# vinits5/bullet-envs

Measured on AMD Instinct MI355X. Metric: env-steps/sec (whole node), 16-link snake, 4096 envs/GPU, higher is better.
Workload: dtype f32

## Files before the change

### bullet-envs_amd/csrc/snk_dynamics.hpp

```cpp
#pragma once
#include "snk_lds.hpp"
#include "snk_model.hpp"
#include "snk_wave.hpp"

namespace snk {

#ifndef SNK_SCALAR_DYNAMICS
__device__ __forceinline__ float quad_yzx(float x) {
    return __int_as_float(__builtin_amdgcn_update_dpp(0, __float_as_int(x), 0xC9, 0xf, 0xf, true));
}
__device__ __forceinline__ float quad_zxy(float x) {
    return __int_as_float(__builtin_amdgcn_update_dpp(0, __float_as_int(x), 0xD2, 0xf, 0xf, true));
}
__device__ __forceinline__ float lane_cross(float a_yzx, float a_zxy, float b) {
#pragma clang fp contract(off)
    return __builtin_fmaf(a_yzx, quad_zxy(b), -(a_zxy * quad_yzx(b)));
}
struct LaneVel {
    float w, v, za, zl;
};
__device__ __forceinline__ LaneVel lane_vel_step(float wp, float vp, float ax, float rb, float qdb) {
#pragma clang fp contract(off)
    const float wy = quad_yzx(wp), wz = quad_zxy(wp);
    const float cr = lane_cross(wy, wz, rb);
    LaneVel o;
    o.w = __builtin_fmaf(ax, qdb, wp);
    o.v = vp + cr;
    o.za = lane_cross(wy, wz, ax) * qdb;
    o.zl = lane_cross(wy, wz, cr);
    return o;
}
#endif

template <class LT>
__device__ void fk_vel(LT& L, const DevModel& M, int lane) {
    constexpr int N = LT::kN;
    const float* bs = L.base();
    float qx = bs[3], qy = bs[4], qz = bs[5], qw = bs[6];
    float dd = qx * qx + qy * qy + qz * qz + qw * qw;
    float s2 = 2.0f / dd;
    float xs = qx * s2, ys = qy * s2, zs = qz * s2;
    float wx = qw * xs, wy = qw * ys, wz = qw * zs;
    float xx = qx * xs, xy = qx * ys, xz = qx * zs, yy = qy * ys, yz = qy * zs, zz = qz * zs;
    float Rp[9] = {1 - (yy + zz), xy - wz, xz + wy, xy + wz, 1 - (xx + zz), yz - wx, xz - wy, yz + wx, 1 - (xx + yy)};
    f3 op = ld3(bs), wp = ld3(bs + 7), vp = ld3(bs + 10);
    if (lane == 0) {
#pragma unroll
        for (int i = 0; i < 9; i++) L.R[0][i] = Rp[i];
        st3(L.o[0], op); st3(L.w[0], wp); st3(L.v[0], vp);
        st3(L.r[0], mk3(0, 0, 0)); st3(L.ax[0], mk3(0, 0, 0));
#pragma unroll
        for (int i = 0; i < 6; i++) L.zeta[0][i] = 0.f;
    }
    float snv = 0.f, csv = 1.f;
    if (lane < N) sincosf(L.q()[lane], &snv, &csv);
#ifndef SNK_SCALAR_DYNAMICS
    const int ln = launder_lane(lane);
    const int c = ln & 3, cc = c < 3 ? c : 2;
    float C0 = c == 0 ? Rp[0] : (c == 1 ? Rp[3] : Rp[6]);
    float C1 = c == 0 ? Rp[1] : (c == 1 ? Rp[4] : Rp[7]);
    float C2 = c == 0 ? Rp[2] : (c == 1 ? Rp[5] : Rp[8]);
    float opv = bs[cc], wpv = bs[7 + cc], vpv = bs[10 + cc];
#pragma unroll 4
    for (int b = 1; b <= N; b++) {
#pragma clang fp contract(off)
        const float* Rf = M.Rfix[b];
        const float* pf = M.pfix[b];
        const float qdb = L.qd()[b - 1];
        const float sn = __int_as_float(__builtin_amdgcn_readlane(__float_as_int(snv), b - 1));
        const float cs = __int_as_float(__builtin_amdgcn_readlane(__float_as_int(csv), b - 1));
        const float T0 = __builtin_fmaf(C2, Rf[6], __builtin_fmaf(C0, Rf[0], C1 * Rf[3]));
        const float T1 = __builtin_fmaf(C2, Rf[7], __builtin_fmaf(C0, Rf[1], C1 * Rf[4]));
        const float T2 = __builtin_fmaf(C2, Rf[8], __builtin_fmaf(C0, Rf[2], C1 * Rf[5]));
        const float N0 = __builtin_fmaf(T0, cs, -(sn * T2));
        const float N2 = __builtin_fmaf(sn, T0, cs * T2);
        const float rb = __builtin_fmaf(C2, pf[2], __builtin_fmaf(C0, pf[0], C1 * pf[1]));
        const float o = opv + rb;
        const LaneVel k = lane_vel_step(wpv, vpv, T1, rb, qdb);
        if (ln < 3) {
            L.R[b][3 * c] = N0; L.R[b][3 * c + 1] = T1; L.R[b][3 * c + 2] = N2;
            L.o[b][c] = o; L.r[b][c] = rb; L.ax[b][c] = T1; L.w[b][c] = k.w; L.v[b][c] = k.v;
            L.zeta[b][c] = k.za; L.zeta[b][3 + c] = k.zl;
        }
        C0 = N0; C1 = T1; C2 = N2;
        opv = o; wpv = k.w; vpv = k.v;
    }
#else
#pragma unroll 4
    for (int b = 1; b <= N; b++) {
        const float* Rf = M.Rfix[b];
        float T[9];
#pragma unroll
        for (int i = 0; i < 3; i++)
#pragma unroll
            for (int j = 0; j < 3; j++)
                T[3 * i + j] = Rp[3 * i] * Rf[j] + Rp[3 * i + 1] * Rf[3 + j] + Rp[3 * i + 2] * Rf[6 + j];
        float qdb = L.qd()[b - 1];
        const float sn = __int_as_float(__builtin_amdgcn_readlane(__float_as_int(snv), b - 1));
        const float cs = __int_as_float(__builtin_amdgcn_readlane(__float_as_int(csv), b - 1));
        float Rn[9];
#pragma unroll
        for (int i = 0; i < 3; i++) {
            Rn[3 * i + 0] = cs * T[3 * i] - sn * T[3 * i + 2];
            Rn[3 * i + 1] = T[3 * i + 1];
            Rn[3 * i + 2] = sn * T[3 * i] + cs * T[3 * i + 2];
        }
        f3 rb = mulRv(Rp, ld3(M.pfix[b]));
        f3 o = op + rb;
        f3 ax = mk3(T[1], T[4], T[7]);
        f3 w = wp + ax * qdb;
        f3 v = vp + cross(wp, rb);
        f3 za = cross(wp, ax) * qdb;
        f3 zl = cross(wp, cross(wp, rb));
        if (lane == 0) {
#pragma unroll
            for (int i = 0; i < 9; i++) L.R[b][i] = Rn[i];
            st3(L.o[b], o); st3(L.r[b], rb); st3(L.ax[b], ax); st3(L.w[b], w); st3(L.v[b], v);
            st3(&L.zeta[b][0], za); st3(&L.zeta[b][3], zl);
        }
#pragma unroll
        for (int i = 0; i < 9; i++) Rp[i] = Rn[i];
        op = o; wp = w; vp = v;
    }
#endif
    lds_sync();
}

template <class LT>
__device__ __forceinline__ void vel_refresh(LT& L, int lane) {
    constexpr int N = LT::kN;
#ifdef SNK_SCALAR_DYNAMICS
    f3 wp = ld3(L.base() + 7), vp = ld3(L.base() + 10);
    if (lane == 0) { st3(L.w[0], wp); st3(L.v[0], vp); }
    for (int b = 1; b <= N; b++) {
        f3 ax = ld3(L.ax[b]), rb = ld3(L.r[b]);
        float qdb = L.qd()[b - 1];
        f3 w = wp + ax * qdb, v = vp + cross(wp, rb);
        f3 za = cross(wp, ax) * qdb, zl = cross(wp, cross(wp, rb));
        if (lane == 0) { st3(L.w[b], w); st3(L.v[b], v); st3(&L.zeta[b][0], za); st3(&L.zeta[b][3], zl); }
        wp = w; vp = v;
    }
#else
    const int ln = launder_lane(lane);
    const int c = ln & 3, cc = c < 3 ? c : 2;
    float wpv = L.base()[7 + cc], vpv = L.base()[10 + cc];
    if (ln < 3) { L.w[0][c] = wpv; L.v[0][c] = vpv; }
    for (int b = 1; b <= N; b++) {
        const LaneVel k = lane_vel_step(wpv, vpv, L.ax[b][cc], L.r[b][cc], L.qd()[b - 1]);
        if (ln < 3) { L.w[b][c] = k.w; L.v[b][c] = k.v; L.zeta[b][c] = k.za; L.zeta[b][3 + c] = k.zl; }
        wpv = k.w; vpv = k.v;
    }
#endif
}

template <class LT>
__device__ float mean_height(LT& L, const DevModel& M, int lane) {
    constexpr int N = LT::kN;
    float z = 0.f;
    if (lane == 0) z = L.o[0][2] + L.R[0][6] * M.hbase[0] + L.R[0][7] * M.hbase[1] + L.R[0][8] * M.hbase[2];
    else if (lane <= N) z = L.o[lane][2];
    return wave_sum<64>(z) * (1.0f / (N + 1));
}

template <class LT, bool FIRST>
__device__ void body_bias(LT& L, const DevModel& M, int lane) {
    constexpr int N = LT::kN;
    if (lane <= N) {
        const int b = lane;
        const float* R = L.R[b];
        f3 w = ld3(L.w[b]), v = ld3(L.v[b]);
        float m = M.mass[b];
        f3 cw = mulRv(R, ld3(M.com[b]));
        float Ibar[6];
        rotSym(R, M.Ib[b], Ibar);
        f3 pN = cross(w, mulSv(Ibar, w));
        f3 pF = cross(w, cross(w, cw)) * m;
        float Irw[6];
        rotSym(R, M.Irot[b], Irw);
        float nw = sqrtf(dot(w, w));
        pN = pN + mulSv(Irw, w) * (M.ang_damp + M.ang_damp * nw);
        const int ns = M.nsub[b];
        for (int s = 0; s < ns; s++) {
            f3 cs = mulRv(R, ld3(M.sub_c[b][s]));
            f3 vs = v + cross(w, cs);
            float nv = sqrtf(dot(vs, vs));
            f3 F = vs * (M.sub_m[b][s] * (M.lin_damp + M.lin_damp * nv));
            pF = pF + F;
            pN = pN + cross(cs, F);
        }
        if (FIRST) {
            f3 G = mk3(0.f, 0.f, m * M.gz);
            pF = pF - G;
            pN = pN - cross(cw, G);
            st3(L.cw[b], cw);
            float* IA = L.IA[b];
#pragma unroll
            for (int i = 0; i < 6; i++) IA[i] = Ibar[i];
            float hx = m * cw.x, hy = m * cw.y, hz = m * cw.z;
            IA[6] = 0.f; IA[7] = -hz; IA[8] = hy;
            IA[9] = hz;  IA[10] = 0.f; IA[11] = -hx;
            IA[12] = -hy; IA[13] = hx; IA[14] = 0.f;
            IA[15] = m; IA[16] = 0.f; IA[17] = 0.f; IA[18] = m; IA[19] = 0.f; IA[20] = m;
        } else {
            pN = pN - ld3(L.ext(b));
            pF = pF - ld3(L.ext(b) + 3);
        }
        st3(&L.p[b][0], pN);
        st3(&L.p[b][3], pF);
    }
}

template <class LT, bool FACTOR>
__device__ void aba_main(LT& L, const DevModel& M, int lane
#ifdef SNK_PROFILE_FINE
                         , unsigned long long* prof_f = nullptr
#endif
) {
    constexpr int N = LT::kN;
    float cA[6], cB[9], cC[6];
#pragma unroll
    for (int i = 0; i < 6; i++) { cA[i] = 0.f; cC[i] = 0.f; }
#pragma unroll
    for (int i = 0; i < 9; i++) cB[i] = 0.f;
    f3 cN = mk3(0, 0, 0), cF = mk3(0, 0, 0);
    for (int b = N; b >= 1; b--) {
        float A[6], B[9], C[6];
        float* IA = L.IA[b];
#pragma unroll
        for (int i = 0; i < 6; i++) { A[i] = IA[i]; C[i] = IA[15 + i]; }
#pragma unroll
        for (int i = 0; i < 9; i++) B[i] = IA[6 + i];
        if (FACTOR) {
#pragma unroll
            for (int i = 0; i < 6; i++) { A[i] += cA[i]; C[i] += cC[i]; }
#pragma unroll
            for (int i = 0; i < 9; i++) B[i] += cB[i];
        }
        f3 pN = ld3(&L.p[b][0]) + cN, pF = ld3(&L.p[b][3]) + cF;
        f3 ax = ld3(L.ax[b]);
        f3 Ua, Ub;
        float Dinv;
        if (FACTOR) {
            Ua = mulSv(A, ax);
            Ub = mk3(B[0] * ax.x + B[3] * ax.y + B[6] * ax.z, B[1] * ax.x + B[4] * ax.y + B[7] * ax.z,
                     B[2] * ax.x + B[5] * ax.y + B[8] * ax.z);
            Dinv = 1.0f / dot(ax, Ua);
        } else {
            Ua = ld3(L.Ua[b]); Ub = ld3(L.Ub[b]); Dinv = L.Dinv[b];
        }
        f3 za = ld3(&L.zeta[b][0]), zl = ld3(&L.zeta[b][3]);
        float u = L.tauj[b - 1] - dot(ax, pN);
        f3 tN = mulSv(A, za) + mk3(B[0] * zl.x + B[1] * zl.y + B[2] * zl.z, B[3] * zl.x + B[4] * zl.y + B[5] * zl.z,
                                   B[6] * zl.x + B[7] * zl.y + B[8] * zl.z);
        f3 tF = mk3(B[0] * za.x + B[3] * za.y + B[6] * za.z, B[1] * za.x + B[4] * za.y + B[7] * za.z,
                    B[2] * za.x + B[5] * za.y + B[8] * za.z) + mulSv(C, zl);
        float uz = dot(Ua, za) + dot(Ub, zl);
        float s = (u - uz) * Dinv;
        f3 paN = pN + tN + Ua * s, paF = pF + tF + Ub * s;
        f3 r = ld3(L.r[b]);
        cN = paN + cross(r, paF);
        cF = paF;
        if (lane == 0) {
            L.u[b] = u;
            if (FACTOR) {
#pragma unroll
                for (int i = 0; i < 6; i++) { IA[i] = A[i]; IA[15 + i] = C[i]; }
#pragma unroll
                for (int i = 0; i < 9; i++) IA[6 + i] = B[i];
                st3(L.Ua[b], Ua); st3(L.Ub[b], Ub); L.Dinv[b] = Dinv;
            }
        }
        if (FACTOR) {
            float ua[3] = {Ua.x, Ua.y, Ua.z}, ub[3] = {Ub.x, Ub.y, Ub.z};
            float Ap[6], Bp[9], Cp[6];
            Ap[0] = A[0] - ua[0] * ua[0] * Dinv; Ap[1] = A[1] - ua[0] * ua[1] * Dinv; Ap[2] = A[2] - ua[0] * ua[2] * Dinv;
            Ap[3] = A[3] - ua[1] * ua[1] * Dinv; Ap[4] = A[4] - ua[1] * ua[2] * Dinv; Ap[5] = A[5] - ua[2] * ua[2] * Dinv;
            Cp[0] = C[0] - ub[0] * ub[0] * Dinv; Cp[1] = C[1] - ub[0] * ub[1] * Dinv; Cp[2] = C[2] - ub[0] * ub[2] * Dinv;
            Cp[3] = C[3] - ub[1] * ub[1] * Dinv; Cp[4] = C[4] - ub[1] * ub[2] * Dinv; Cp[5] = C[5] - ub[2] * ub[2] * Dinv;
#pragma unroll
            for (int i = 0; i < 3; i++)
#pragma unroll
                for (int j = 0; j < 3; j++) Bp[3 * i + j] = B[3 * i + j] - ua[i] * ub[j] * Dinv;
            f3 c0 = cross(r, mk3(Cp[0], Cp[1], Cp[2]));
            f3 c1 = cross(r, mk3(Cp[1], Cp[3], Cp[4]));
            f3 c2 = cross(r, mk3(Cp[2], Cp[4], Cp[5]));
            float Bn[9] = {Bp[0] + c0.x, Bp[1] + c1.x, Bp[2] + c2.x, Bp[3] + c0.y, Bp[4] + c1.y, Bp[5] + c2.y,
                           Bp[6] + c0.z, Bp[7] + c1.z, Bp[8] + c2.z};
            f3 e0 = cross(r, mk3(Bp[0], Bp[1], Bp[2])), e1 = cross(r, mk3(Bp[3], Bp[4], Bp[5])),
               e2 = cross(r, mk3(Bp[6], Bp[7], Bp[8]));
            f3 g0 = cross(r, mk3(Bn[0], Bn[1], Bn[2])), g1 = cross(r, mk3(Bn[3], Bn[4], Bn[5])),
               g2 = cross(r, mk3(Bn[6], Bn[7], Bn[8]));
            cA[0] = Ap[0] + e0.x + g0.x;
            cA[1] = Ap[1] + e0.y + g1.x;
            cA[2] = Ap[2] + e0.z + g2.x;
            cA[3] = Ap[3] + e1.y + g1.y;
            cA[4] = Ap[4] + e1.z + g2.y;
            cA[5] = Ap[5] + e2.z + g2.z;
#pragma unroll
            for (int i = 0; i < 9; i++) cB[i] = Bn[i];
#pragma unroll
            for (int i = 0; i < 6; i++) cC[i] = Cp[i];
        }
    }
    SNK_FSTAMP(2)
    f3 pN = ld3(&L.p[0][0]) + cN, pF = ld3(&L.p[0][3]) + cF;
    float p0[6] = {pN.x, pN.y, pN.z, pF.x, pF.y, pF.z};
    if (FACTOR) {
        float* IA = L.IA[0];
        float A[6], B[9], C[6];
#pragma unroll
        for (int i = 0; i < 6; i++) { A[i] = IA[i] + cA[i]; C[i] = IA[15 + i] + cC[i]; }
#pragma unroll
        for (int i = 0; i < 9; i++) B[i] = IA[6 + i] + cB[i];
        float G[6][6];
        G[0][0] = A[0]; G[0][1] = A[1]; G[0][2] = A[2]; G[1][1] = A[3]; G[1][2] = A[4]; G[2][2] = A[5];
        G[1][0] = A[1]; G[2][0] = A[2]; G[2][1] = A[4];
        G[3][3] = C[0]; G[3][4] = C[1]; G[3][5] = C[2]; G[4][4] = C[3]; G[4][5] = C[4]; G[5][5] = C[5];
        G[4][3] = C[1]; G[5][3] = C[2]; G[5][4] = C[4];
#pragma unroll
        for (int i = 0; i < 3; i++)
#pragma unroll
            for (int j = 0; j < 3; j++) { G[i][3 + j] = B[3 * i + j]; G[3 + j][i] = B[3 * i + j]; }
        float V[6][6];
#pragma unroll
        for (int i = 0; i < 6; i++)
#pragma unroll
            for (int j = 0; j < 6; j++) V[i][j] = (i == j) ? 1.f : 0.f;
#pragma unroll
        for (int k = 0; k < 6; k++) {
            float piv = 1.0f / G[k][k];
#pragma unroll
            for (int j = 0; j < 6; j++) { G[k][j] *= piv; V[k][j] *= piv; }
#pragma unroll
            for (int i = 0; i < 6; i++) {
                if (i != k) {
                    float f = G[i][k];
#pragma unroll
                    for (int j = 0; j < 6; j++) { G[i][j] -= f * G[k][j]; V[i][j] -= f * V[k][j]; }
                }
            }
        }
        if (lane == 0) {
#pragma unroll
            for (int i = 0; i < 6; i++)
#pragma unroll
                for (int j = 0; j < 6; j++) L.Inv0[6 * i + j] = V[i][j];
        }
        float a0[6];
#pragma unroll
        for (int i = 0; i < 6; i++) {
            float s = 0.f;
#pragma unroll
            for (int j = 0; j < 6; j++) s -= V[i][j] * p0[j];
            a0[i] = s;
        }
        if (lane == 0) {
#pragma unroll
            for (int i = 0; i < 6; i++) L.acc0[i] = a0[i];
        }
    } else {
        float a0[6];
#pragma unroll
        for (int i = 0; i < 6; i++) {
            float s = 0.f;
#pragma unroll
            for (int j = 0; j < 6; j++) s -= L.Inv0[6 * i + j] * p0[j];
            a0[i] = s;
        }
        if (lane == 0) {
#pragma unroll
            for (int i = 0; i < 6; i++) L.acc0[i] = a0[i];
        }
    }
    lds_sync();
    SNK_FSTAMP(3)
    if (!FACTOR) return;
    f3 al = ld3(&L.acc0[0]), a = ld3(&L.acc0[3]);
    for (int b = 1; b <= N; b++) {
        f3 r = ld3(L.r[b]);
        f3 ap = a + cross(al, r) + ld3(&L.zeta[b][3]);
        f3 alp = al + ld3(&L.zeta[b][0]);
        float qdd = (L.u[b] - (dot(ld3(L.Ua[b]), alp) + dot(ld3(L.Ub[b]), ap))) * L.Dinv[b];
        al = alp + ld3(L.ax[b]) * qdd;
        a = ap;
        if (lane == 0) L.qdd[b - 1] = qdd;
    }
    lds_sync();
    SNK_FSTAMP(4)
}

template <class LT>
__device__ __forceinline__ bool sensor_pass_needed(LT& L, const DevModel& M, int lane, float dv, const SensorHint& hint) {
    constexpr int N = LT::kN;
    constexpr int ND = N + 6;
    if (hint.always) return true;
    const float dt = M.dt;
    float e = 0.f, wgt = 0.f;
    if (lane < ND) {
        const float vold = lane < 6 ? L.base()[7 + lane] : L.qd()[lane - 6];
        const float x = fminf(fmaxf(vold + dv, -M.max_vel), M.max_vel);
        if (lane >= 6) e = L.targets[lane - 6] - (L.q()[lane - 6] + dt * x);
        const int m = N + 5 - lane;
        const float arm = lane < 3 ? (M.reach_hb + M.reach_l * (0.5f * N * (N + 1))) * (1.0f / (N + 1))
                                   : (lane < 6 ? 1.0f : M.reach_l * ((float)(m * (m + 1)) * (0.5f / (N + 1))));
        wgt = fabsf(x) * arm;
    }
    const float se = wave_sum<64>(e * e);
    const float reach = dt * wave_sum<64>(wgt) + kReachSlack;
    const float tol = M.servo_tol * 1.001f;
    const bool sensor = !(se > tol * tol) || hint.counter_next > M.max_counter || !(hint.h_prev + reach < M.height_thr);
    return __builtin_amdgcn_readfirstlane(sensor ? 1 : 0) != 0;
}

}
```

Baseline: 376,100.

## Lane-parallelize ABA backward sweep across quad lanes with DPP broadcasts

Rewrites the articulated-body backward pass so each of the first three lanes in a quad owns one row/column of the 3x3 inertia blocks, using DPP quad broadcasts to exchange values instead of each lane computing the full 6x6 update redundantly. It also writes the updated articulated inertia back to LDS in the factor case and uses a wavefront fence. This cuts per-lane arithmetic and register pressure in the serial link recursion, at the cost of more cross-lane permutes, extra LDS writes and a more intricate, error-prone index scheme.

```diff
diff --git a/bullet-envs_amd/csrc/snk_dynamics.hpp b/bullet-envs_amd/csrc/snk_dynamics.hpp
--- a/bullet-envs_amd/csrc/snk_dynamics.hpp
+++ b/bullet-envs_amd/csrc/snk_dynamics.hpp
@@ -11,6 +11,10 @@
 }
 __device__ __forceinline__ float quad_zxy(float x) {
     return __int_as_float(__builtin_amdgcn_update_dpp(0, __float_as_int(x), 0xD2, 0xf, 0xf, true));
+}
+template <int K>
+__device__ __forceinline__ float quad_bcast(float x) {
+    return __int_as_float(__builtin_amdgcn_update_dpp(0, __float_as_int(x), K * 0x55, 0xf, 0xf, true));
 }
 __device__ __forceinline__ float lane_cross(float a_yzx, float a_zxy, float b) {
 #pragma clang fp contract(off)
@@ -223,6 +227,106 @@
 #pragma unroll
     for (int i = 0; i < 9; i++) cB[i] = 0.f;
     f3 cN = mk3(0, 0, 0), cF = mk3(0, 0, 0);
+#ifndef SNK_SCALAR_DYNAMICS
+    {
+        const int ln = launder_lane(lane);
+        const int c = ln & 3, cc = c < 3 ? c : 2;
+        const int s1 = cc == 0 ? 1 : cc + 2, s2 = cc == 0 ? 2 : cc + 3;
+        const int cy = cc == 2 ? 0 : cc + 1, cz = cc == 0 ? 2 : cc - 1;
+        float a0 = 0.f, a1 = 0.f, a2 = 0.f;
+        float h0 = 0.f, h1 = 0.f, h2 = 0.f;
+        float d0 = 0.f, d1 = 0.f, d2 = 0.f;
+        float cNv = 0.f, cFv = 0.f;
+#pragma unroll 4
+        for (int b = N; b >= 1; b--) {
+#pragma clang fp contract(off)
+            float* IA = L.IA[b];
+            float A0 = IA[cc], A1 = IA[s1], A2 = IA[s2];
+            float H0 = IA[6 + 3 * cc], H1 = IA[7 + 3 * cc], H2 = IA[8 + 3 * cc];
+            float D0 = IA[15 + cc], D1 = IA[15 + s1], D2 = IA[15 + s2];
+            if (FACTOR) {
+                A0 += a0; A1 += a1; A2 += a2; H0 += h0; H1 += h1; H2 += h2; D0 += d0; D1 += d1; D2 += d2;
+                if (ln < 3) {
+                    IA[cc] = A0; IA[s1] = A1; IA[s2] = A2;
+                    IA[6 + 3 * cc] = H0; IA[7 + 3 * cc] = H1; IA[8 + 3 * cc] = H2;
+                    IA[15 + cc] = D0; IA[15 + s1] = D1; IA[15 + s2] = D2;
+                }
+                __builtin_amdgcn_fence(__ATOMIC_ACQ_REL, "wavefront");
+            }
+            const float K0 = IA[6 + cc], K1 = IA[9 + cc], K2 = IA[12 + cc];
+            const float pNv = L.p[b][cc] + cNv, pFv = L.p[b][3 + cc] + cFv;
+            const f3 ax = ld3(L.ax[b]);
+            float Uav, Ubv, Dinv;
+            f3 Ua, Ub;
+            if (FACTOR) {
+                Uav = __builtin_fmaf(A2, ax.z, __builtin_fmaf(A0, ax.x, A1 * ax.y));
+                Ubv = __builtin_fmaf(K2, ax.z, __builtin_fmaf(K0, ax.x, K1 * ax.y));
+                Ua = mk3(quad_bcast<0>(Uav), quad_bcast<1>(Uav), quad_bcast<2>(Uav));
+                Ub = mk3(quad_bcast<0>(Ubv), quad_bcast<1>(Ubv), quad_bcast<2>(Ubv));
+                Dinv = 1.0f / __builtin_fmaf(ax.z, Ua.z, __builtin_fmaf(ax.x, Ua.x, ax.y * Ua.y));
+            } else {
+                Ua = ld3(L.Ua[b]); Ub = ld3(L.Ub[b]); Dinv = L.Dinv[b];
+                Uav = L.Ua[b][cc]; Ubv = L.Ub[b][cc];
+            }
+            const f3 za = ld3(&L.zeta[b][0]), zl = ld3(&L.zeta[b][3]);
+            const float pNx = quad_bcast<0>(pNv), pNy = quad_bcast<1>(pNv), pNz = quad_bcast<2>(pNv);
+            const float u = L.tauj[b - 1] - __builtin_fmaf(pNz, ax.z, __builtin_fmaf(pNx, ax.x, pNy * ax.y));
+            const float tNv = __builtin_fmaf(A2, za.z, __builtin_fmaf(A0, za.x, A1 * za.y)) +
+                              __builtin_fmaf(H2, zl.z, __builtin_fmaf(H0, zl.x, H1 * zl.y));
+            const float tFv = __builtin_fmaf(K2, za.z, __builtin_fmaf(K0, za.x, K1 * za.y)) +
+                              __builtin_fmaf(D2, zl.z, __builtin_fmaf(D0, zl.x, D1 * zl.y));
+            const float uz = __builtin_fmaf(Ua.z, za.z, __builtin_fmaf(Ua.x, za.x, Ua.y * za.y)) +
+                             __builtin_fmaf(Ub.z, zl.z, __builtin_fmaf(Ub.x, zl.x, Ub.y * zl.y));
+            const float s = Dinv * (u - uz);
+            const float paNv = __builtin_fmaf(Uav, s, pNv + tNv), paFv = __builtin_fmaf(Ubv, s, pFv + tFv);
+            const float ry = L.r[b][cy], rz = L.r[b][cz];
+            cNv = paNv + lane_cross(ry, rz, paFv);
+            cFv = paFv;
+            if (ln < 3) {
+                L.u[b] = u;
+                if (FACTOR) { L.Ua[b][cc] = Uav; L.Ub[b][cc] = Ubv; L.Dinv[b] = Dinv; }
+            }
+            if (FACTOR) {
+                const f3 r = ld3(L.r[b]);
+                const float Ap0 = __builtin_fmaf(-(Uav * Ua.x), Dinv, A0), Ap1 = __builtin_fmaf(-(Uav * Ua.y), Dinv, A1),
+                            Ap2 = __builtin_fmaf(-(Uav * Ua.z), Dinv, A2);
+                const float Cp0 = __builtin_fmaf(-(Ubv * Ub.x), Dinv, D0), Cp1 = __builtin_fmaf(-(Ubv * Ub.y), Dinv, D1),
+                            Cp2 = __builtin_fmaf(-(Ubv * Ub.z), Dinv, D2);
+                const float P0 = __builtin_fmaf(-(Uav * Ub.x), Dinv, H0), P1 = __builtin_fmaf(-(Uav * Ub.y), Dinv, H1),
+                            P2 = __builtin_fmaf(-(Uav * Ub.z), Dinv, H2);
+                const float y1 = quad_zxy(Cp1), z1 = quad_yzx(Cp1);
+                const float w1 = __builtin_fmaf(ry, y1, -(rz * z1)), w1o = __builtin_fmaf(-z1, rz, y1 * ry);
+                h0 = P0 + lane_cross(ry, rz, Cp0);
+                h1 = P1 + (cc == 1 ? w1o : w1);
+                h2 = P2 + lane_cross(ry, rz, Cp2);
+                const float e0 = __builtin_fmaf(P2, r.y, -(P1 * r.z)), e1 = __builtin_fmaf(P0, r.z, -(r.x * P2)),
+                            e2 = __builtin_fmaf(r.x, P1, -(P0 * r.y));
+                const float g0 = __builtin_fmaf(r.y, h2, -(r.z * h1)), g1 = __builtin_fmaf(r.z, h0, -(r.x * h2)),
+                            g2 = __builtin_fmaf(r.x, h1, -(r.y * h0));
+                const float g10 = quad_bcast<1>(g0), g20 = quad_bcast<2>(g0), g21 = quad_bcast<2>(g1);
+                const float n0 = (Ap0 + e0) + g0;
+                const float n1 = (Ap1 + e1) + (cc == 0 ? g10 : g1);
+                const float n2 = (Ap2 + e2) + (cc == 0 ? g20 : (cc == 1 ? g21 : g2));
+                const float m01 = quad_bcast<0>(n1), m02 = quad_bcast<0>(n2), m12 = quad_bcast<1>(n2);
+                a0 = cc == 0 ? n0 : (cc == 1 ? m01 : m02);
+                a1 = cc == 2 ? m12 : n1;
+                a2 = n2;
+                d0 = Cp0; d1 = Cp1; d2 = Cp2;
+            }
+        }
+        cN = mk3(quad_bcast<0>(cNv), quad_bcast<1>(cNv), quad_bcast<2>(cNv));
+        cF = mk3(quad_bcast<0>(cFv), quad_bcast<1>(cFv), quad_bcast<2>(cFv));
+        if (FACTOR) {
+            cA[0] = quad_bcast<0>(a0); cA[1] = quad_bcast<0>(a1); cA[2] = quad_bcast<0>(a2);
+            cA[3] = quad_bcast<1>(a1); cA[4] = quad_bcast<1>(a2); cA[5] = quad_bcast<2>(a2);
+            cC[0] = quad_bcast<0>(d0); cC[1] = quad_bcast<0>(d1); cC[2] = quad_bcast<0>(d2);
+            cC[3] = quad_bcast<1>(d1); cC[4] = quad_bcast<1>(d2); cC[5] = quad_bcast<2>(d2);
+            cB[0] = quad_bcast<0>(h0); cB[1] = quad_bcast<0>(h1); cB[2] = quad_bcast<0>(h2);
+            cB[3] = quad_bcast<1>(h0); cB[4] = quad_bcast<1>(h1); cB[5] = quad_bcast<1>(h2);
+            cB[6] = quad_bcast<2>(h0); cB[7] = quad_bcast<2>(h1); cB[8] = quad_bcast<2>(h2);
+        }
+    }
+#else
     for (int b = N; b >= 1; b--) {
         float A[6], B[9], C[6];
         float* IA = L.IA[b];
@@ -302,6 +406,7 @@
             for (int i = 0; i < 6; i++) cC[i] = Cp[i];
         }
     }
+#endif
     SNK_FSTAMP(2)
     f3 pN = ld3(&L.p[0][0]) + cN, pF = ld3(&L.p[0][3]) + cF;
     float p0[6] = {pN.x, pN.y, pN.z, pF.x, pF.y, pF.z};
```

Result: no change. 378,000 (median of 6 runs) (+0.5%).
